# Maboroshi0327/MHAda-Style-Transfer

Hardware: AMD Instinct MI355X
Metric: stylized frames/sec (whole job) at 512x512 batch 8 fp32 [configs[1]] (higher is better)
Workload: dtype f32; 1 GPU; stylize 512x512 content+style, batch 8; resolution=512, batch_per_gpu=8, global_batch=8, compute_dtype=f32, parallelism=replicas x1

## Files before the change

mhada-style-transfer_amd/csrc/abi.hip:

```cpp
#include "common.h"

#include <mutex>
#include <stdlib.h>
#include <string.h>

namespace mhada {

static thread_local std::string g_last_error;

void set_error(const std::string& msg) { g_last_error = msg; }

int fail(const std::string& msg) {
  set_error(msg);
  return MHADA_ERR_ARG;
}

int check_launch(const char* what) {
  const hipError_t e = hipGetLastError();
  if (e != hipSuccess) {
    set_error(std::string(what) + ": " + hipGetErrorString(e));
    return MHADA_ERR_LAUNCH;
  }
  return MHADA_OK;
}

namespace {
struct Knob {
  const char* name;
  int Tuning::*field;
};
const Knob kKnobs[] = {
    {"attn_fixed_shift", &Tuning::attn_fixed_shift}, {"attn_waves", &Tuning::attn_waves},
    {"attn_tk", &Tuning::attn_tk},                   {"attn_prio", &Tuning::attn_prio},
    {"vit_attn_vec", &Tuning::vit_attn_vec},         {"out3_mfma", &Tuning::out3_mfma},
    {"out3_tile", &Tuning::out3_tile},               {"gemm_pp", &Tuning::gemm_pp},
    {"gemm_persist", &Tuning::gemm_persist},         {"gemm_pp128", &Tuning::gemm_pp128},
    {"gemm_ldsepi", &Tuning::gemm_ldsepi},           {"gemm_n64", &Tuning::gemm_n64},
    {"conv_c64", &Tuning::conv_c64},                 {"conv_dir", &Tuning::conv_dir},                 {"gemm_rinit", &Tuning::gemm_rinit},
    {"tn_skinny_lds", &Tuning::tn_skinny_lds},       {"train_dkv_dma", &Tuning::train_dkv_dma},
    {"wino_split3", &Tuning::wino_split3},
    {"wino4", &Tuning::wino4},                       {"upsample_quad", &Tuning::upsample_quad},
    {"xknob", &Tuning::xknob},
};

Tuning g_tuning;
std::once_flag g_tuning_once;

void read_env_once() {
  std::call_once(g_tuning_once, [] {
    for (const Knob& k : kKnobs) {
      std::string env = "MHADA_";
      for (const char* c = k.name; *c; ++c) env += (char)(*c >= 'a' && *c <= 'z' ? *c - 32 : *c);
      if (const char* v = getenv(env.c_str())) g_tuning.*k.field = atoi(v);
    }
  });
}

bool valid(const char* name, int v) {
  if (!strcmp(name, "attn_waves")) return v == 0 || v == 4 || v == 8;
  if (!strcmp(name, "attn_tk")) return v == 64 || v == 128;
  if (!strcmp(name, "gemm_n64")) return v == 128 || v == 256;
  if (!strcmp(name, "xknob")) return v >= 0 && v < 16;
  return v == 0 || v == 1;
}
}

const Tuning& tuning() {
  read_env_once();
  return g_tuning;
}

}

extern "C" int mhada_abi_version(void) { return 17; }

extern "C" const char* mhada_last_error(void) { return mhada::g_last_error.c_str(); }

extern "C" int mhada_set_tuning(const char* name, int value) {
  using namespace mhada;
  read_env_once();
  if (!name) return fail("mhada_set_tuning: null name");
  for (const Knob& k : kKnobs) {
    if (!strcmp(k.name, name)) {
      if (!valid(name, value)) return fail(std::string("mhada_set_tuning: bad value for ") + name);
      g_tuning.*k.field = value;
      return MHADA_OK;
    }
  }
  return fail(std::string("mhada_set_tuning: unknown knob ") + name);
}

extern "C" int mhada_get_tuning(const char* name, int* value) {
  using namespace mhada;
  read_env_once();
  if (!name || !value) return fail("mhada_get_tuning: null argument");
  for (const Knob& k : kKnobs) {
    if (!strcmp(k.name, name)) {
      *value = g_tuning.*k.field;
      return MHADA_OK;
    }
  }
  return fail(std::string("mhada_get_tuning: unknown knob ") + name);
}
```

mhada-style-transfer_amd/csrc/common.h:

```cpp
#pragma once
#include <hip/hip_runtime.h>
#include <stdint.h>
#include <string>

#include "../../include/mhada_hip.h"

typedef __bf16 bf16;
typedef __bf16 bf16x8 __attribute__((ext_vector_type(8)));
typedef __bf16 bf16x4 __attribute__((ext_vector_type(4)));
typedef float f32x16 __attribute__((ext_vector_type(16)));
typedef float f32x4 __attribute__((ext_vector_type(4)));
typedef float f32x2 __attribute__((ext_vector_type(2)));

#define MHADA_DEV __device__ __forceinline__

namespace mhada {

void set_error(const std::string& msg);
int fail(const std::string& msg);
int check_launch(const char* what);

struct Tuning {
  int attn_fixed_shift = 1;
  int attn_waves = 0;
  int attn_tk = 128;
  int attn_prio = 1;
  int vit_attn_vec = 1;
  int out3_mfma = 1;
  int out3_tile = 1;
  int gemm_pp = 1;
  int gemm_persist = 1;
  int gemm_pp128 = 1;
  int gemm_ldsepi = 1;
  int gemm_n64 = 128;
  int conv_c64 = 1;
  int conv_dir = 1;
  int gemm_rinit = 1;
  int tn_skinny_lds = 1;
  int wino4 = 1;
  int wino_split3 = 1;
  int train_dkv_dma = 1;
  int upsample_quad = 1;
  int xknob = 0;
};
const Tuning& tuning();

int conv3x3_c64(const void* x, const void* w, const float* bias, void* y, int B, int H, int W, bool up, int relu,
                hipStream_t s);
int conv3x3_dir(const void* x, const void* w, const float* bias, void* y, int B, int H, int W, int cin, int cout,
                int relu, hipStream_t s);

template <typename T> MHADA_DEV float to_f32(T x);
template <> MHADA_DEV float to_f32<float>(float x) { return x; }
template <> MHADA_DEV float to_f32<bf16>(bf16 x) { return (float)x; }

template <typename T> MHADA_DEV T from_f32(float x);
template <> MHADA_DEV float from_f32<float>(float x) { return x; }
template <> MHADA_DEV bf16 from_f32<bf16>(float x) { return (bf16)x; }

template <typename T> struct Vec16;
template <> struct Vec16<float> { typedef f32x4 type; static constexpr int N = 4; };
template <> struct Vec16<bf16> { typedef bf16x8 type; static constexpr int N = 8; };

MHADA_DEV float bilerp(float ly0, float ly1, float lx0, float lx1, float x00, float x01, float x10, float x11) {
  return fmaf(ly1, fmaf(lx0, x10, lx1 * x11), ly0 * fmaf(lx0, x00, lx1 * x01));
}

MHADA_DEV float wave_sum(float v) {
#pragma unroll
  for (int o = 32; o > 0; o >>= 1) v += __shfl_xor(v, o, 64);
  return v;
}
MHADA_DEV float wave_max(float v) {
#pragma unroll
  for (int o = 32; o > 0; o >>= 1) v = fmaxf(v, __shfl_xor(v, o, 64));
  return v;
}

MHADA_DEV int xcd_remap(int bid, int nblk) {
  const int q = nblk / 8, r = nblk % 8;
  const int xcd = bid % 8, k = bid / 8;
  return (xcd < r ? xcd * (q + 1) : r * (q + 1) + (xcd - r) * q) + k;
}

}
```

mhada-style-transfer_amd/csrc/gemm_impl.h:

```cpp
#pragma once
#include "common.h"

#include <algorithm>
#include <mutex>
#include <stdlib.h>

namespace mhada {

struct GemmP {
  int M, N, K, nb2;
  const void* a; long long lda, sa1, sa2;
  const float* a_mu; long long smu1, smu2;
  int img_c, img_h, img_w, out_h, out_w;
  int pad;
  const void* w; long long ldw, sw1, sw2;
  const float* bias; long long sb1, sb2;
  const void* r; long long ldr, sr1, sr2;
  void* c; long long ldc, sc1, sc2;
  int relu, tiles_n, ntiles;
  int lds_epi;
  int rinit;
  void* c2; long long ldc2, sc21, sc22;
  void* vt; long long ldt, svt1, svt2;
  long long spl;
// ... 731 lines not shown
  for (int a = 0; a < 4; ++a)
#pragma unroll
    for (int b = 0; b < 2; ++b)
#pragma unroll
      for (int e = 0; e < 16; ++e) acc[a][b][e] = 0.f;
  auto compute = [&](int nt) {
    __builtin_amdgcn_s_setprio(1);
#pragma unroll
    for (int s2 = 0; s2 < 2; ++s2)
#pragma unroll
      for (int mt = 0; mt < 4; ++mt)
        acc[mt][nt] = __builtin_amdgcn_mfma_f32_32x32x16_bf16(wf[nt][s2], af[mt][s2], acc[mt][nt], 0, 0, 0);
    __builtin_amdgcn_s_setprio(0);
  };

  const int KT = p.K / BK;
  stage_a(0, 0); stage_a(1, 0); stage_w(0, 0); stage_w(1, 0);
  if (KT > 1) {
    stage_a(0, 1); stage_a(1, 1);
    asm volatile("s_waitcnt vmcnt(4)" ::: "memory");
  } else {
    asm volatile("s_waitcnt vmcnt(0)" ::: "memory");
  }
  PP_BARRIER();
  if (grp == 1) PP_BARRIER();

  for (int kt = 0; kt < KT; ++kt) {
    const int cb = kt & 1;
    const bool n1 = kt + 1 < KT, n2 = kt + 2 < KT;
    read_a(0, cb); read_w(0, 0, cb);
    if (n1) stage_w(0, kt + 1);
    PP_LGKM0(); PP_BARRIER(); compute(0); PP_BARRIER();
    read_w(1, 0, cb);
    if (n1) stage_w(1, kt + 1);
    PP_LGKM0(); PP_BARRIER(); compute(1); PP_BARRIER();
    read_a(1, cb); read_w(0, 1, cb);
    PP_LGKM0(); PP_BARRIER(); compute(0); PP_BARRIER();
    read_w(1, 1, cb);
    if (n2) {
      stage_a(0, kt + 2); stage_a(1, kt + 2);
      asm volatile("s_waitcnt vmcnt(4)" ::: "memory");
    } else {
      asm volatile("s_waitcnt vmcnt(0)" ::: "memory");
    }
    PP_LGKM0(); PP_BARRIER(); compute(1); PP_BARRIER();
  }
  if (grp == 0) PP_BARRIER();
  store_tile<TO, 4, 2>(p, acc, z1, z2, m0 + grp * 128 + r32, n0 + wc * 64, h);
}

template <typename TC, typename TO, int AMODE, int BN>
__global__ void __launch_bounds__(512) gemm_ppp_kernel(const GemmP p, int total) {
  constexpr int TN = BN / 128, NWH = BN / 128;
  constexpr int CE = 16 / sizeof(TC), BK = 8 * CE, PE = 1024 / sizeof(TC), HALF = 128 * BK, TILE = (2 + NWH) * HALF;
  constexpr int NSLOT = BN == 256 ? 2 : 3;
  typedef typename Vec16<TC>::type Frag;
  constexpr int SCR = BN == 256 ? 8 * 4096 / (int)sizeof(TC) : 0;
  __shared__ __attribute__((aligned(16))) TC smem[NSLOT * TILE + SCR];
  const int tid = threadIdx.x, lane = tid & 63;
  const int wave = __builtin_amdgcn_readfirstlane(tid >> 6);
  const int grp = wave >> 2, wc = wave & 3;
  const int h = lane >> 5, r32 = lane & 31;
  const int G = gridDim.x;

  int cofs[2];
#pragma unroll
  for (int i = 0; i < 2; ++i) cofs[i] = CE * ((lane & 7) ^ (4 * i + (lane >> 4)));
  struct St {
    const TC* ab;
    const TC* wb;
    unsigned aoff[2][2], woff[2][2];
    int b[2][2], y[2][2], x[2][2];
    int m0, n0, z1, z2;
  };
  auto setup = [&](int w, St& s) {
    const int lg = xcd_remap(w, total);
    const int z = lg / p.ntiles, t = lg - z * p.ntiles;
    s.z1 = z / p.nb2;
    s.z2 = z - s.z1 * p.nb2;
    const int tm = t / p.tiles_n, tn = t - tm * p.tiles_n;
    s.m0 = tm * 256;
    s.n0 = tn * BN;
    s.ab = reinterpret_cast<const TC*>(p.a) + s.z1 * p.sa1 + s.z2 * p.sa2;
    s.wb = reinterpret_cast<const TC*>(p.w) + s.z1 * p.sw1 + s.z2 * p.sw2;
#pragma unroll
    for (int hh = 0; hh < 2; ++hh)
#pragma unroll
      for (int i = 0; i < 2; ++i) {
        const int rr = 16 * wave + 8 * i + (lane >> 3);
        const int m = min(s.m0 + 128 * hh + rr, p.M - 1);
        const int n = min(s.n0 + 128 * (hh % NWH) + rr, p.N - 1);
        s.woff[hh][i] = (unsigned)((long long)n * p.ldw + cofs[i]);
        if constexpr (AMODE == MHADA_A_ROWS || AMODE == kRowsSplit3) {
          s.aoff[hh][i] = (unsigned)((long long)m * p.lda + cofs[i]);
        } else {
          const int hw = p.out_h * p.out_w;
          const int b = m / hw, rem = m - b * hw;
          s.b[hh][i] = b;
          s.y[hh][i] = rem / p.out_w;
          s.x[hh][i] = rem - (rem / p.out_w) * p.out_w;
          s.aoff[hh][i] = 0;
        }
      }
  };
  auto stage_a = [&](const St& s, int hh, int kt, int slot) {
    TC* dst = smem + slot * TILE + hh * HALF + wave * 2 * PE;
    const int k0 = kt * BK;
    if constexpr (AMODE == MHADA_A_ROWS) {
#pragma unroll
      for (int i = 0; i < 2; ++i) glds16(s.ab + s.aoff[hh][i] + k0, dst + PE * i);
    } else if constexpr (AMODE == kRowsSplit3) {
      const int kk = kt / 6, t = kt - 6 * kk;
      const TC* src = s.ab + ((kSplitPlanes >> (4 * t)) & 15) * p.spl + kk * BK;
#pragma unroll
      for (int i = 0; i < 2; ++i) glds16(src + s.aoff[hh][i], dst + PE * i);
    } else {
      const int cin_n = p.img_c;
      const int tap = k0 / cin_n, cin0 = k0 - tap * cin_n;
      const int dy = tap / 3 - 1, dx = tap - (tap / 3) * 3 - 1;
#pragma unroll
      for (int i = 0; i < 2; ++i) {
        int Y, X;
        const bool inside = conv_src<AMODE>(p, s.y[hh][i], s.x[hh][i], dy, dx, Y, X);
        const unsigned off = (unsigned)(((s.b[hh][i] * p.img_h + Y) * p.img_w + X) * cin_n + cin0 + cofs[i]);
        glds16(inside ? (const void*)(s.ab + off) : (const void*)g_zero16, dst + PE * i);
      }
    }
  };
  auto stage_w = [&](const St& s, int hh, int kt, int slot) {
    TC* dst = smem + slot * TILE + (2 + hh) * HALF + wave * 2 * PE;
#pragma unroll
    for (int i = 0; i < 2; ++i) glds16(s.wb + s.woff[hh][i] + kt * BK, dst + PE * i);
  };

  const int swz = (r32 >> 1) & 7;
  int koff[4];
#pragma unroll
  for (int ks = 0; ks < 4; ++ks) koff[ks] = sizeof(TC) == 2 ? CE * ((2 * ks + h) ^ swz) : CE * ((4 * h + ks) ^ swz);
  const TC* sA = smem + grp * HALF + r32 * BK;
  const TC* sW = smem + (2 + (wc * TN * 32) / 128) * HALF + ((wc * TN * 32) % 128 + r32) * BK;
  Frag af[4][2], wf[TN][2];
  auto read_a = [&](int kp, int cb) {
#pragma unroll
    for (int mt = 0; mt < 4; ++mt)
#pragma unroll
      for (int s2 = 0; s2 < 2; ++s2)
        af[mt][s2] = *reinterpret_cast<const Frag*>(sA + cb * TILE + mt * 32 * BK + koff[2 * kp + s2]);
  };
  auto read_w = [&](int nt, int kp, int cb) {
#pragma unroll
    for (int s2 = 0; s2 < 2; ++s2)
      wf[nt][s2] = *reinterpret_cast<const Frag*>(sW + cb * TILE + nt * 32 * BK + koff[2 * kp + s2]);
  };
  f32x16 acc[4][TN];
  auto zero_acc = [&](const St& s) {
    if constexpr (sizeof(TO) == 4) {
      if (p.rinit) {
        const float* rb = reinterpret_cast<const float*>(p.r) + s.z1 * p.sr1 + s.z2 * p.sr2;
        const float* bb = p.bias ? p.bias + s.z1 * p.sb1 + s.z2 * p.sb2 : nullptr;
#pragma unroll
        for (int nt = 0; nt < TN; ++nt)
#pragma unroll
          for (int g = 0; g < 4; ++g) {
            const int n = s.n0 + wc * TN * 32 + nt * 32 + 8 * g + 4 * h;
            const bool nok = n + 3 < p.N;
            const f32x4 b4 = (bb && nok) ? *reinterpret_cast<const f32x4*>(bb + n) : f32x4{0.f, 0.f, 0.f, 0.f};
#pragma unroll
            for (int mt = 0; mt < 4; ++mt) {
              const int m = s.m0 + grp * 128 + mt * 32 + r32;
              f32x4 r4 = {0.f, 0.f, 0.f, 0.f};
              if (nok && m < p.M) r4 = *reinterpret_cast<const f32x4*>(rb + (long long)m * p.ldr + n);
#pragma unroll
              for (int e = 0; e < 4; ++e) acc[mt][nt][4 * g + e] = r4[e] + b4[e];
            }
          }
        return;
      }
    }
#pragma unroll
    for (int a = 0; a < 4; ++a)
#pragma unroll
      for (int b = 0; b < TN; ++b)
#pragma unroll
        for (int e = 0; e < 16; ++e) acc[a][b][e] = 0.f;
  };
  GemmP pe = p;
  if (p.rinit) {
    pe.r = nullptr;
    pe.bias = nullptr;
  }
  auto compute = [&](int nt) {
    __builtin_amdgcn_s_setprio(1);
    if constexpr (sizeof(TC) == 2) {
#pragma unroll
      for (int s2 = 0; s2 < 2; ++s2)
#pragma unroll
        for (int mt = 0; mt < 4; ++mt)
          acc[mt][nt] = __builtin_amdgcn_mfma_f32_32x32x16_bf16(wf[nt][s2], af[mt][s2], acc[mt][nt], 0, 0, 0);
    } else {
#pragma unroll
      for (int s2 = 0; s2 < 2; ++s2)
#pragma unroll
        for (int e = 0; e < 4; ++e)
#pragma unroll
          for (int mt = 0; mt < 4; ++mt)
            acc[mt][nt] = __builtin_amdgcn_mfma_f32_32x32x2f32(wf[nt][s2][e], af[mt][s2][e], acc[mt][nt], 0, 0, 0);
    }
    __builtin_amdgcn_s_setprio(0);
  };

  const int KT = p.K / BK;
  int w = blockIdx.x;
  St cur, nxt;
  setup(w, cur);
  bool has_nxt = w + G < total;
  if (has_nxt) setup(w + G, nxt);
  zero_acc(cur);
  stage_a(cur, 0, 0, 0); stage_a(cur, 1, 0, 0); stage_w(cur, 0, 0, 0);
  if constexpr (NWH == 2) stage_w(cur, 1, 0, 0);
  stage_a(cur, 0, 1, 1); stage_a(cur, 1, 1, 1);
  asm volatile("s_waitcnt vmcnt(4)" ::: "memory");
  PP_BARRIER();
  if (grp == 1) PP_BARRIER();

  int sl0 = 0, sl1 = 1, sl2 = NSLOT == 2 ? 0 : 2;
  constexpr int EPI_MIN = (sizeof(TO) == 4 && TN == 2) ? 32 : 16;
  auto ktile = [&](const St& s1, const int k1, const bool w1, const St& s2, const int k2, const bool a2,
                   const bool wx) __attribute__((always_inline)) {
    const int cb = sl0;
    if constexpr (TN == 2) {
      read_a(0, cb); read_w(0, 0, cb);
      if (w1) stage_w(s1, 0, k1, sl1);
      PP_LGKM0(); PP_BARRIER(); compute(0); PP_BARRIER();
      read_w(1, 0, cb);
      if (w1) stage_w(s1, 1, k1, sl1);
      PP_LGKM0(); PP_BARRIER(); compute(1); PP_BARRIER();
      read_a(1, cb); read_w(0, 1, cb);
      PP_LGKM0(); PP_BARRIER(); compute(0); PP_BARRIER();
      read_w(1, 1, cb);
    } else {
      read_a(0, cb); read_w(0, 0, cb);
      if (w1) stage_w(s1, 0, k1, sl1);
      PP_LGKM0(); PP_BARRIER(); compute(0); PP_BARRIER();
      read_a(1, cb); read_w(0, 1, cb);
    }
    if (a2) {
      stage_a(s2, 0, k2, sl2); stage_a(s2, 1, k2, sl2);
      if (wx) asm volatile("s_waitcnt vmcnt(%0)" :: "n"(4 + EPI_MIN) : "memory");
      else asm volatile("s_waitcnt vmcnt(4)" ::: "memory");
    } else {
      asm volatile("s_waitcnt vmcnt(0)" ::: "memory");
    }
    PP_LGKM0(); PP_BARRIER(); compute(TN - 1); PP_BARRIER();
    if constexpr (NSLOT == 2) {
      sl0 ^= 1; sl1 ^= 1; sl2 ^= 1;
    } else {
      const int o = sl0;
      sl0 = sl1; sl1 = sl2; sl2 = o;
    }
  };
  bool pre = false;
  while (true) {
    if constexpr (AMODE == MHADA_A_ROWS || AMODE == kRowsSplit3) {
      for (int kt = 0; kt + 2 < KT; ++kt) ktile(cur, kt + 1, kt > 0 || !pre, cur, kt + 2, true, kt == 0 && pre);
      ktile(cur, KT - 1, KT > 2 || !pre, nxt, 0, has_nxt, KT == 2 && pre);
    } else {
      for (int kt = 0; kt + 2 < KT; ++kt) ktile(cur, kt + 1, true, cur, kt + 2, true, false);
      ktile(cur, KT - 1, true, nxt, 0, has_nxt, false);
    }
    ktile(nxt, 0, has_nxt, nxt, 1, has_nxt, false);
    if (grp == 0) PP_BARRIER();
    pre = (AMODE == MHADA_A_ROWS || AMODE == kRowsSplit3) && has_nxt && !p.rinit && cur.m0 + 256 <= p.M &&
          cur.n0 + BN <= p.N;
    if (pre) {
      stage_w(nxt, 0, 1, sl1);
      if constexpr (NWH == 2) stage_w(nxt, 1, 1, sl1);
    }
    __builtin_amdgcn_sched_barrier(0);
    if constexpr (SCR > 0) {
      if (p.lds_epi) {
        float* scr = reinterpret_cast<float*>(smem + NSLOT * TILE) + wave * 1024;
        if constexpr (sizeof(TO) == 2 && TN == 2) {
          store_tile_lds_bf16<4>(pe, acc, cur.z1, cur.z2, cur.m0 + grp * 128, cur.n0 + wc * TN * 32, lane, scr);
        } else {
          store_tile_lds<TO, 4, TN, AMODE == kRowsSplit3>(pe, acc, cur.z1, cur.z2, cur.m0 + grp * 128,
                                                           cur.n0 + wc * TN * 32, lane, scr);
        }
      }
      else
        store_tile<TO, 4, TN>(pe, acc, cur.z1, cur.z2, cur.m0 + grp * 128 + r32, cur.n0 + wc * TN * 32, h);
    } else {
      store_tile<TO, 4, TN>(pe, acc, cur.z1, cur.z2, cur.m0 + grp * 128 + r32, cur.n0 + wc * TN * 32, h);
    }
    if (!has_nxt) break;
    if (grp == 1) PP_BARRIER();
    zero_acc(nxt);
    cur = nxt;
    w += G;
    has_nxt = w + G < total;
    if (has_nxt) setup(w + G, nxt);
  }
}

template <int BM, int NS, int BK>
__global__ void __launch_bounds__(BM * 2) gemm_n64_kernel(const GemmP p) {
  constexpr int NWV = BM / 32, CH = BK / 4, RPI = 64 / CH;
  constexpr int AH = BM * BK, WH = 64 * BK, STAGE = AH + WH;
  constexpr int API = 32 / RPI, WPI = 64 / RPI / NWV;
  static_assert(WPI >= 1 && (CH == 8 || CH == 16), "tile config");
  __shared__ __attribute__((aligned(16))) float smem[NS * STAGE];
  const int tid = threadIdx.x, lane = tid & 63;
  const int wave = __builtin_amdgcn_readfirstlane(tid >> 6);
  int z, tile;
  if (p.lds_epi == 4) {
    const int L = blockIdx.y * gridDim.x + blockIdx.x, nt = gridDim.x;
    z = L % 8 + 8 * (L / (8 * nt));
    tile = (L / 8) % nt;
  } else {
    z = blockIdx.y;
    tile = xcd_remap(blockIdx.x, p.ntiles);
  }
  const int z1 = z / p.nb2, z2 = z - z1 * p.nb2;
  const int m0 = tile * BM;
  const float* ab = reinterpret_cast<const float*>(p.a) + z1 * p.sa1 + z2 * p.sa2;
  const float* wb = reinterpret_cast<const float*>(p.w) + z1 * p.sw1 + z2 * p.sw2;
  auto sw = [](int r) { return CH == 8 ? (r >> 1) & 7 : r & 15; };
  const float* asrc[API];
  const float* wsrc[WPI];
#pragma unroll
  for (int i = 0; i < API; ++i) {
    const int r = 32 * wave + RPI * i + lane / CH;
    const int m = min(m0 + r, p.M - 1);
    asrc[i] = ab + (long long)m * p.lda + 4 * ((lane % CH) ^ sw(r));
  }
#pragma unroll
  for (int i = 0; i < WPI; ++i) {
    const int r = RPI * (WPI * wave + i) + lane / CH;
    const int n = min(r, p.N - 1);
    wsrc[i] = wb + (long long)n * p.ldw + 4 * ((lane % CH) ^ sw(r));
  }
  auto stage = [&](int kt, int slot) {
    float* dst = smem + slot * STAGE;
    const int k0 = kt * BK;
#pragma unroll
    for (int i = 0; i < API; ++i) glds16(asrc[i] + k0, dst + (32 * wave + RPI * i) * BK);
#pragma unroll
    for (int i = 0; i < WPI; ++i) glds16(wsrc[i] + k0, dst + AH + RPI * (WPI * wave + i) * BK);
  };
  const int h = lane >> 5, r32 = lane & 31;
  int koff[CH / 2];
#pragma unroll
  for (int q = 0; q < CH / 2; ++q) koff[q] = 4 * (((CH / 2) * h + q) ^ sw(r32));
  f32x16 acc[1][2];
#pragma unroll
  for (int n = 0; n < 2; ++n)
#pragma unroll
    for (int e = 0; e < 16; ++e) acc[0][n][e] = 0.f;
  const int KT = p.K / BK;
#pragma unroll
  for (int i = 0; i < NS - 1; ++i)
    if (i < KT) stage(i, i);
  for (int kt = 0; kt < KT; ++kt) {
    const int ahead = min(KT - 1 - kt, NS - 2);
    if (ahead >= 2) asm volatile("s_waitcnt vmcnt(%0)" :: "n"(2 * (API + WPI)) : "memory");
    else if (ahead == 1) asm volatile("s_waitcnt vmcnt(%0)" :: "n"(API + WPI) : "memory");
    else asm volatile("s_waitcnt vmcnt(0)" ::: "memory");
    PP_BARRIER();
    if (kt + NS - 1 < KT) stage(kt + NS - 1, (kt + NS - 1) % NS);
    const float* sa = smem + (kt % NS) * STAGE + (32 * wave + r32) * BK;
    const float* swp = smem + (kt % NS) * STAGE + AH + r32 * BK;
    f32x4 af[CH / 2], wf[2][CH / 2];
#pragma unroll
    for (int q = 0; q < CH / 2; ++q) af[q] = *reinterpret_cast<const f32x4*>(sa + koff[q]);
#pragma unroll
    for (int n = 0; n < 2; ++n)
#pragma unroll
      for (int q = 0; q < CH / 2; ++q) wf[n][q] = *reinterpret_cast<const f32x4*>(swp + n * 32 * BK + koff[q]);
#pragma unroll
    for (int s = 0; s < BK / 2; ++s)
#pragma unroll
      for (int n = 0; n < 2; ++n)
        acc[0][n] = __builtin_amdgcn_mfma_f32_32x32x2f32(wf[n][s >> 2][s & 3], af[s >> 2][s & 3], acc[0][n], 0, 0, 0);
  }
  store_tile<float, 1, 2>(p, acc, z1, z2, m0 + 32 * wave + r32, 0, h);
}

static bool aligned16(const void* ptr) { return ((uintptr_t)ptr & 15) == 0; }

static int num_cus() {
  static int n = 0;
  if (!n) {
    int dev = 0;
    (void)hipGetDevice(&dev);
    if (hipDeviceGetAttribute(&n, hipDeviceAttributeMultiprocessorCount, dev) != hipSuccess || n <= 0) n = 256;
  }
  return n;
}

static bool persist_enabled() { return tuning().gemm_persist != 0; }

template <typename TC, typename TO, int AMODE, int BN = 256>
static int launch_gemm_pp(const GemmP& p0, int nz, hipStream_t stream) {
  GemmP p = p0;
  p.tiles_n = (p.N + BN - 1) / BN;
  p.ntiles = ((p.M + 255) / 256) * p.tiles_n;
  p.lds_epi = tuning().gemm_ldsepi ? 1 : 0;
  p.rinit = (sizeof(TO) == 4 && p.r && !p.relu && tuning().gemm_rinit && ((uintptr_t)p.r & 15) == 0 &&
             p.ldr % 4 == 0 && p.sr1 % 4 == 0 && p.sr2 % 4 == 0 && p.N % 4 == 0) ? 1 : 0;
  const long long total = (long long)p.ntiles * nz;
  if (sizeof(TC) == 4 || BN != 256 || AMODE == kRowsSplit3 || (p.K >= 128 && persist_enabled() && total < (1LL << 31))) {
    const int grid = (int)std::min<long long>(total, num_cus());
    hipLaunchKernelGGL((gemm_ppp_kernel<TC, TO, AMODE, BN>), dim3(grid), dim3(512), 0, stream, p, (int)total);
    return check_launch("mhada_gemm");
  }
  if constexpr (sizeof(TC) == 2 && BN == 256 && AMODE != kRowsSplit3) {
    hipLaunchKernelGGL((gemm_pp_kernel<TO, AMODE>), dim3(p.ntiles, nz), dim3(512), 0, stream, p);
    return check_launch("mhada_gemm");
  }
  return fail("mhada_gemm: no ping-pong form");
}

static bool pp_enabled() { return tuning().gemm_pp != 0; }

template <typename TC, typename TA, typename TO, int AMODE, int BM, int BN, int WM, int WN>
static int launch_gemm(const GemmP& p0, int nz, hipStream_t stream) {
  GemmP p = p0;
  p.tiles_n = (p.N + BN - 1) / BN;
  p.lds_epi = (tuning().gemm_ldsepi &&
               (size_t)2 * (BM + BN) * Cfg<TC>::LS * sizeof(TC) >= (size_t)WM * WN * 4096) ? 1 : 0;
  const int tiles_m = (p.M + BM - 1) / BM;
  p.ntiles = tiles_m * p.tiles_n;
  const size_t lds2 = (size_t)2 * (BM + BN) * Cfg<TC>::LS * sizeof(TC);
  const size_t lds = p.K > Cfg<TC>::BK ? lds2
                                       : std::max(lds2 / 2, (size_t)(p.lds_epi || p.vt ? WM * WN * 4096 : 0));
  static std::once_flag attr_once;
  std::call_once(attr_once, [&] {
    (void)hipFuncSetAttribute((const void*)gemm_kernel<TC, TA, TO, AMODE, BM, BN, WM, WN>,
                              hipFuncAttributeMaxDynamicSharedMemorySize, (int)lds2);
  });
  hipLaunchKernelGGL((gemm_kernel<TC, TA, TO, AMODE, BM, BN, WM, WN>), dim3(p.ntiles, nz), dim3(64 * WM * WN),
                     lds, stream, p);
  return check_launch("mhada_gemm");
}

static bool pp_offsets_fit(const GemmP& p, int amode) {
  const long long lim = 1LL << 31;
  const long long wspan = (long long)(p.N - 1) * p.ldw + p.K;
  long long aspan;
  if (amode == MHADA_A_ROWS) aspan = (long long)(p.M - 1) * p.lda + p.K;
  else aspan = (long long)p.M / ((long long)p.out_h * p.out_w) * p.img_h * p.img_w * p.img_c;
  return wspan < lim && aspan < lim;
}

template <typename TC, typename TA, typename TO, int AMODE>
static int dispatch_tile(const GemmP& p, int nz, hipStream_t s) {
  if constexpr (AMODE == MHADA_A_ROWS || AMODE == kRowsCentred) {
    if (p.vt) {
      if constexpr (sizeof(TC) == 2) return launch_gemm<TC, TA, TO, AMODE, 256, 128, 4, 2>(p, nz, s);
      else return launch_gemm<TC, TA, TO, AMODE, 128, 128, 2, 2>(p, nz, s);
    }
  }
  if (p.N <= 64) {
    if constexpr (sizeof(TC) == 4 && sizeof(TA) == 4 && sizeof(TO) == 4 && AMODE == MHADA_A_ROWS) {
      if (p.K % 32 == 0 && p.lda % 4 == 0 && p.ldw % 4 == 0 && p.sa1 % 4 == 0 && p.sa2 % 4 == 0 &&
          p.sw1 % 4 == 0 && p.sw2 % 4 == 0 && aligned16(p.a) && aligned16(p.w)) {
        GemmP q = p;
        q.tiles_n = 1;
        q.lds_epi = nz % 8 == 0 ? 4 : 0;
        if (p.K >= 1024 && p.K % 64 == 0) {
          q.ntiles = (p.M + 255) / 256;
          hipLaunchKernelGGL((gemm_n64_kernel<256, 2, 64>), dim3(q.ntiles, nz), dim3(512), 0, s, q);
        } else {
          q.ntiles = (p.M + 127) / 128;
          hipLaunchKernelGGL((gemm_n64_kernel<128, 2, 32>), dim3(q.ntiles, nz), dim3(256), 0, s, q);
        }
        return check_launch("mhada_gemm");
      }
    }
    if (tuning().gemm_n64 == 256) return launch_gemm<TC, TA, TO, AMODE, 256, 64, 8, 1>(p, nz, s);
    return launch_gemm<TC, TA, TO, AMODE, 128, 64, 4, 1>(p, nz, s);
  }
  if constexpr (sizeof(TC) == 4) {
    if constexpr (sizeof(TA) == 4 && (AMODE == MHADA_A_ROWS || AMODE == MHADA_A_CONV3X3 || AMODE == MHADA_A_CONV3X3_ZERO)) {
      const long long t256 = (long long)((p.M + 255) / 256) * ((p.N + 255) / 256) * nz;
      if (p.N > 128 && p.K % 32 == 0 && p.K >= 64 && 8 * t256 >= 7LL * num_cus() && pp_enabled() && persist_enabled() &&
          pp_offsets_fit(p, AMODE)) {
        return launch_gemm_pp<float, TO, AMODE>(p, nz, s);
      }
    }
    return launch_gemm<TC, TA, TO, AMODE, 128, 128, 2, 2>(p, nz, s);
  } else {
    if constexpr (AMODE == MHADA_A_CONV3X3_UP2) {
      return launch_gemm<TC, TA, TO, AMODE, 128, 128, 2, 2>(p, nz, s);
    } else {
      if constexpr (sizeof(TA) == 2 && (AMODE == MHADA_A_ROWS || AMODE == MHADA_A_CONV3X3)) {
        if (p.N > 128 && p.K % 64 == 0 && pp_enabled() && pp_offsets_fit(p, AMODE))
          return launch_gemm_pp<bf16, TO, AMODE>(p, nz, s);
        if (p.N > 64 && p.N <= 128 && p.K % 64 == 0 && p.K >= 128 && tuning().gemm_pp128 && pp_enabled() &&
            pp_offsets_fit(p, AMODE))
          return launch_gemm_pp<bf16, TO, AMODE, 128>(p, nz, s);
      }
      if (p.N <= 128) return launch_gemm<TC, TA, TO, AMODE, 256, 128, 4, 2>(p, nz, s);
      return launch_gemm<TC, TA, TO, AMODE, 256, 256, 2, 4>(p, nz, s);
    }
  }
}

template <typename TC, typename TA, typename TO>
static int dispatch_mode(int mode, const GemmP& p, int nz, hipStream_t s) {
  switch (mode) {
    case MHADA_A_ROWS:
      if (p.a_mu) return dispatch_tile<TC, TA, TO, kRowsCentred>(p, nz, s);
      return dispatch_tile<TC, TA, TO, MHADA_A_ROWS>(p, nz, s);
    case MHADA_A_CONV3X3: return dispatch_tile<TC, TA, TO, MHADA_A_CONV3X3>(p, nz, s);
    case MHADA_A_CONV3X3_UP2: return dispatch_tile<TC, TA, TO, MHADA_A_CONV3X3_UP2>(p, nz, s);
    case MHADA_A_CONV3X3_ZERO: return dispatch_tile<TC, TA, TO, MHADA_A_CONV3X3_ZERO>(p, nz, s);
    case MHADA_A_PATCH8:
      if constexpr (sizeof(TA) == 4) return dispatch_tile<TC, TA, TO, MHADA_A_PATCH8>(p, nz, s);
      return fail("mhada_gemm: PATCH8 needs an fp32 image");
    case MHADA_A_SPLIT3:
      if constexpr (sizeof(TC) == 2 && sizeof(TA) == 2) {
        if (nz != 1 || p.N <= 128 || p.K % (6 * 64) || p.K < 6 * 64 || !pp_offsets_fit(p, MHADA_A_ROWS))
          return fail("mhada_gemm: SPLIT3 needs one problem, N > 128, K0 = K / 6 a multiple of 64 and 32-bit offsets");
        return launch_gemm_pp<bf16, TO, kRowsSplit3>(p, nz, s);
      }
      return fail("mhada_gemm: SPLIT3 needs bf16 planes and bf16 compute");
  }
  return fail("mhada_gemm: bad a_mode");
}



int gemm_dispatch_f32(int mode, const GemmP& p, int nz, hipStream_t s);
int gemm_dispatch_bf16_a32_o32(int mode, const GemmP& p, int nz, hipStream_t s);
int gemm_dispatch_bf16_a32_o16(int mode, const GemmP& p, int nz, hipStream_t s);
int gemm_dispatch_bf16_a16_o32(int mode, const GemmP& p, int nz, hipStream_t s);
int gemm_dispatch_bf16_a16_o16(int mode, const GemmP& p, int nz, hipStream_t s);

}
```

Before: 335.6 frames/s.

## Add dedicated split-3 row GEMM kernel with reordered A/W staging schedule

Adds a persistent bf16 GEMM kernel for the split-3 row A-mode (used by Winograd/conv lowering). Each 6-block K chunk reuses A planes across weight blocks through a custom ktile ordering, so global-to-LDS loads for A and W are interleaved with MFMA compute on double-buffered slots. It is enabled by default through a new gemm_s3_order knob when nz==1. The hand-tuned vmcnt waits and barrier sequencing are intricate and could go wrong on edge shapes, for example when K is not a multiple of 384.

```diff
diff --git a/mhada-style-transfer_amd/csrc/abi.hip b/mhada-style-transfer_amd/csrc/abi.hip
--- a/mhada-style-transfer_amd/csrc/abi.hip
+++ b/mhada-style-transfer_amd/csrc/abi.hip
@@ -38,7 +38,7 @@
     {"gemm_ldsepi", &Tuning::gemm_ldsepi},           {"gemm_n64", &Tuning::gemm_n64},
     {"conv_c64", &Tuning::conv_c64},                 {"conv_dir", &Tuning::conv_dir},                 {"gemm_rinit", &Tuning::gemm_rinit},
     {"tn_skinny_lds", &Tuning::tn_skinny_lds},       {"train_dkv_dma", &Tuning::train_dkv_dma},
-    {"wino_split3", &Tuning::wino_split3},
+    {"wino_split3", &Tuning::wino_split3},           {"gemm_s3_order", &Tuning::gemm_s3_order},
     {"wino4", &Tuning::wino4},                       {"upsample_quad", &Tuning::upsample_quad},
     {"xknob", &Tuning::xknob},
 };
diff --git a/mhada-style-transfer_amd/csrc/common.h b/mhada-style-transfer_amd/csrc/common.h
--- a/mhada-style-transfer_amd/csrc/common.h
+++ b/mhada-style-transfer_amd/csrc/common.h
@@ -39,6 +39,7 @@
   int tn_skinny_lds = 1;
   int wino4 = 1;
   int wino_split3 = 1;
+  int gemm_s3_order = 1;
   int train_dkv_dma = 1;
   int upsample_quad = 1;
   int xknob = 0;
diff --git a/mhada-style-transfer_amd/csrc/gemm_impl.h b/mhada-style-transfer_amd/csrc/gemm_impl.h
--- a/mhada-style-transfer_amd/csrc/gemm_impl.h
+++ b/mhada-style-transfer_amd/csrc/gemm_impl.h
@@ -1057,6 +1057,198 @@
   }
 }
 
+template <typename TO>
+__global__ void __launch_bounds__(512) gemm_s3_kernel(const GemmP p, int total) {
+  constexpr int BK = 64, PE = 512, HALF = 128 * BK, SLOT = 2 * HALF;
+  constexpr int SCR = 8 * 4096 / 2;
+  __shared__ __attribute__((aligned(16))) bf16 smem[4 * SLOT + SCR];
+  bf16* const smA = smem;
+  bf16* const smW = smem + 2 * SLOT;
+  const int tid = threadIdx.x, lane = tid & 63;
+  const int wave = __builtin_amdgcn_readfirstlane(tid >> 6);
+  const int grp = wave >> 2, wc = wave & 3;
+  const int h = lane >> 5, r32 = lane & 31;
+  const int G = gridDim.x;
+
+  int cofs[2];
+#pragma unroll
+  for (int i = 0; i < 2; ++i) cofs[i] = 8 * ((lane & 7) ^ (4 * i + (lane >> 4)));
+  struct St {
+    unsigned aoff[2][2], woff[2][2];
+    int m0, n0;
+  };
+  const bf16* const ab = reinterpret_cast<const bf16*>(p.a);
+  const bf16* const wb = reinterpret_cast<const bf16*>(p.w);
+  auto setup = [&](int w, St& s) {
+    const int t = xcd_remap(w, total);
+    const int tm = t / p.tiles_n, tn = t - tm * p.tiles_n;
+    s.m0 = tm * 256;
+    s.n0 = tn * 256;
+#pragma unroll
+    for (int hh = 0; hh < 2; ++hh)
+#pragma unroll
+      for (int i = 0; i < 2; ++i) {
+        const int rr = 16 * wave + 8 * i + (lane >> 3);
+        const int m = min(s.m0 + 128 * hh + rr, p.M - 1);
+        const int n = min(s.n0 + 128 * hh + rr, p.N - 1);
+        s.woff[hh][i] = (unsigned)((long long)n * p.ldw + cofs[i]);
+        s.aoff[hh][i] = (unsigned)((long long)m * p.lda + cofs[i]);
+      }
+  };
+  auto stage_a = [&](const St& s, int pl, int kk, int slot) {
+    const bf16* src = ab + pl * p.spl + kk * BK;
+    bf16* dst = smA + slot * SLOT + wave * 2 * PE;
+#pragma unroll
+    for (int hh = 0; hh < 2; ++hh)
+#pragma unroll
+      for (int i = 0; i < 2; ++i) glds16(src + s.aoff[hh][i], dst + hh * HALF + PE * i);
+  };
+  auto stage_w = [&](const St& s, int hh, int blk, int kk, int slot) {
+    const bf16* src = wb + (6 * kk + blk) * BK;
+    bf16* dst = smW + slot * SLOT + hh * HALF + wave * 2 * PE;
+#pragma unroll
+    for (int i = 0; i < 2; ++i) glds16(src + s.woff[hh][i], dst + PE * i);
+  };
+
+  const int swz = (r32 >> 1) & 7;
+  int koff[4];
+#pragma unroll
+  for (int ks = 0; ks < 4; ++ks) koff[ks] = 8 * ((2 * ks + h) ^ swz);
+  const bf16* sA = smA + grp * HALF + r32 * BK;
+  const bf16* sW = smW + (wc >> 1) * HALF + ((wc & 1) * 64 + r32) * BK;
+  bf16x8 af[4][2], wf[2][2];
+  auto read_a = [&](int kp, int slot) {
+#pragma unroll
+    for (int mt = 0; mt < 4; ++mt)
+#pragma unroll
+      for (int s2 = 0; s2 < 2; ++s2)
+        af[mt][s2] = *reinterpret_cast<const bf16x8*>(sA + slot * SLOT + mt * 32 * BK + koff[2 * kp + s2]);
+  };
+  auto read_w = [&](int nt, int kp, int slot) {
+#pragma unroll
+    for (int s2 = 0; s2 < 2; ++s2)
+      wf[nt][s2] = *reinterpret_cast<const bf16x8*>(sW + slot * SLOT + nt * 32 * BK + koff[2 * kp + s2]);
+  };
+  f32x16 acc[4][2];
+  auto zero_acc = [&](const St& s) {
+    if constexpr (sizeof(TO) == 4) {
+      if (p.rinit) {
+        const float* rb = reinterpret_cast<const float*>(p.r);
+        const float* bb = p.bias;
+#pragma unroll
+        for (int nt = 0; nt < 2; ++nt)
+#pragma unroll
+          for (int g = 0; g < 4; ++g) {
+            const int n = s.n0 + wc * 64 + nt * 32 + 8 * g + 4 * h;
+            const bool nok = n + 3 < p.N;
+            const f32x4 b4 = (bb && nok) ? *reinterpret_cast<const f32x4*>(bb + n) : f32x4{0.f, 0.f, 0.f, 0.f};
+#pragma unroll
+            for (int mt = 0; mt < 4; ++mt) {
+              const int m = s.m0 + grp * 128 + mt * 32 + r32;
+              f32x4 r4 = {0.f, 0.f, 0.f, 0.f};
+              if (nok && m < p.M) r4 = *reinterpret_cast<const f32x4*>(rb + (long long)m * p.ldr + n);
+#pragma unroll
+              for (int e = 0; e < 4; ++e) acc[mt][nt][4 * g + e] = r4[e] + b4[e];
+            }
+          }
+        return;
+      }
+    }
+#pragma unroll
+    for (int a = 0; a < 4; ++a)
+#pragma unroll
+      for (int b = 0; b < 2; ++b)
+#pragma unroll
+        for (int e = 0; e < 16; ++e) acc[a][b][e] = 0.f;
+  };
+  GemmP pe = p;
+  if (p.rinit) {
+    pe.r = nullptr;
+    pe.bias = nullptr;
+  }
+  auto compute = [&](int nt) {
+    __builtin_amdgcn_s_setprio(1);
+#pragma unroll
+    for (int s2 = 0; s2 < 2; ++s2)
+#pragma unroll
+      for (int mt = 0; mt < 4; ++mt)
+        acc[mt][nt] = __builtin_amdgcn_mfma_f32_32x32x16_bf16(wf[nt][s2], af[mt][s2], acc[mt][nt], 0, 0, 0);
+    __builtin_amdgcn_s_setprio(0);
+  };
+  constexpr int EPI_MIN = sizeof(TO) == 4 ? 32 : 16;
+  auto wait_vm = [&](int keep) __attribute__((always_inline)) {
+    if (keep == 0) asm volatile("s_waitcnt vmcnt(0)" ::: "memory");
+    else if (keep == 4) asm volatile("s_waitcnt vmcnt(4)" ::: "memory");
+    else if (keep == 8) asm volatile("s_waitcnt vmcnt(8)" ::: "memory");
+    else asm volatile("s_waitcnt vmcnt(%0)" :: "n"(8 + EPI_MIN) : "memory");
+  };
+  auto ktile = [&](int as, int ws, bool sw, const St& wt, int wblk, int wkk, int wsl, bool sa, const St& at, int apl,
+                   int akk, int asl, int keep) __attribute__((always_inline)) {
+    read_a(0, as); read_w(0, 0, ws);
+    if (sw) stage_w(wt, 0, wblk, wkk, wsl);
+    PP_LGKM0(); PP_BARRIER(); compute(0); PP_BARRIER();
+    read_w(1, 0, ws);
+    if (sw) stage_w(wt, 1, wblk, wkk, wsl);
+    PP_LGKM0(); PP_BARRIER(); compute(1); PP_BARRIER();
+    read_a(1, as); read_w(0, 1, ws);
+    PP_LGKM0(); PP_BARRIER(); compute(0); PP_BARRIER();
+    read_w(1, 1, ws);
+    if (sa) stage_a(at, apl, akk, asl);
+    wait_vm(keep);
+    PP_LGKM0(); PP_BARRIER(); compute(1); PP_BARRIER();
+  };
+  int ap = 0;
+  auto chunk = [&](const St& sc, int kk, const St& sn, int kn, bool nx, bool wx) __attribute__((always_inline)) {
+    const int a0 = ap, a1 = ap ^ 1;
+    ktile(a0, 0, true, sc, 0, kk, 1, true, sc, 0, kk, a0, wx ? 8 + EPI_MIN : 8);
+    ktile(a1, 0, false, sc, 0, 0, 0, false, sc, 0, 0, 0, 4);
+    ktile(a1, 1, true, sc, 2, kk, 0, nx, sn, 2, kn, a1, nx ? 8 : 4);
+    ktile(a0, 1, false, sc, 0, 0, 0, false, sc, 0, 0, 0, nx ? 4 : 0);
+    ktile(a0, 0, true, sc, 1, kk, 1, false, sc, 0, 0, 0, 0);
+    ktile(a0, 1, nx, sn, 1, kn, 0, nx, sn, 1, kn, a0, nx ? 4 : 0);
+    ap ^= 1;
+  };
+
+  const int KC = p.K / (6 * BK);
+  int w = blockIdx.x;
+  St cur, nxt;
+  setup(w, cur);
+  bool has_nxt = w + G < total;
+  if (has_nxt) setup(w + G, nxt);
+  zero_acc(cur);
+  stage_a(cur, 2, 0, 0);
+  stage_w(cur, 0, 1, 0, 0); stage_w(cur, 1, 1, 0, 0);
+  stage_a(cur, 1, 0, 1);
+  asm volatile("s_waitcnt vmcnt(4)" ::: "memory");
+  PP_BARRIER();
+  if (grp == 1) PP_BARRIER();
+
+  bool lazy = false;
+  while (true) {
+    for (int kk = 0; kk + 1 < KC; ++kk) chunk(cur, kk, cur, kk + 1, true, kk == 0 && lazy);
+    chunk(cur, KC - 1, nxt, 0, has_nxt, KC == 1 && lazy);
+    if (grp == 0) PP_BARRIER();
+    lazy = has_nxt && !p.rinit && cur.m0 + 256 <= p.M && cur.n0 + 256 <= p.N;
+    __builtin_amdgcn_sched_barrier(0);
+    if (p.lds_epi) {
+      float* scr = reinterpret_cast<float*>(smem + 4 * SLOT) + wave * 1024;
+      if constexpr (sizeof(TO) == 2)
+        store_tile_lds_bf16<4>(pe, acc, 0, 0, cur.m0 + grp * 128, cur.n0 + wc * 64, lane, scr);
+      else
+        store_tile_lds<TO, 4, 2, true>(pe, acc, 0, 0, cur.m0 + grp * 128, cur.n0 + wc * 64, lane, scr);
+    } else {
+      store_tile<TO, 4, 2>(pe, acc, 0, 0, cur.m0 + grp * 128 + r32, cur.n0 + wc * 64, h);
+    }
+    if (!has_nxt) break;
+    if (grp == 1) PP_BARRIER();
+    zero_acc(nxt);
+    cur = nxt;
+    w += G;
+    has_nxt = w + G < total;
+    if (has_nxt) setup(w + G, nxt);
+  }
+}
+
 template <int BM, int NS, int BK>
 __global__ void __launch_bounds__(BM * 2) gemm_n64_kernel(const GemmP p) {
   constexpr int NWV = BM / 32, CH = BK / 4, RPI = 64 / CH;
@@ -1163,6 +1355,13 @@
   p.rinit = (sizeof(TO) == 4 && p.r && !p.relu && tuning().gemm_rinit && ((uintptr_t)p.r & 15) == 0 &&
              p.ldr % 4 == 0 && p.sr1 % 4 == 0 && p.sr2 % 4 == 0 && p.N % 4 == 0) ? 1 : 0;
   const long long total = (long long)p.ntiles * nz;
+  if constexpr (AMODE == kRowsSplit3 && sizeof(TC) == 2 && BN == 256) {
+    if (tuning().gemm_s3_order && nz == 1 && total < (1LL << 31)) {
+      const int grid = (int)std::min<long long>(total, num_cus());
+      hipLaunchKernelGGL((gemm_s3_kernel<TO>), dim3(grid), dim3(512), 0, stream, p, (int)total);
+      return check_launch("mhada_gemm");
+    }
+  }
   if (sizeof(TC) == 4 || BN != 256 || AMODE == kRowsSplit3 || (p.K >= 128 && persist_enabled() && total < (1LL << 31))) {
     const int grid = (int)std::min<long long>(total, num_cus());
     hipLaunchKernelGGL((gemm_ppp_kernel<TC, TO, AMODE, BN>), dim3(grid), dim3(512), 0, stream, p, (int)total);
```

Result: faster. 343.5 frames/s (median of 6 runs) (+2.3%).
